# Raiden-Makoto/MLX-VAE

Hardware: AMD Instinct MI355X
Metric: SELFIES sequences/sec (whole node), AR-CVAE training step (higher is better)
Workload: dtype f32

## Files before the change

### include/arcvae_hip.h

```cpp
#ifndef ARCVAE_HIP_H
#define ARCVAE_HIP_H

#include <stdint.h>

#ifdef __cplusplus
extern "C" {
#endif

#define ARCVAE_OK 0
#define ARCVAE_ERR_ARG (-1)
#define ARCVAE_ERR_LAUNCH (-2)
#define ARCVAE_ERR_DEVICE (-3)

#define ARCVAE_GEMM_ACCUMULATE 1
#define ARCVAE_GEMM_TANH 2
#define ARCVAE_GEMM_SPLITK 4
#define ARCVAE_GEMM_NO_SKINNY 8
#define ARCVAE_GEMM_TILE64 16
#define ARCVAE_GEMM_TILE128 32
#define ARCVAE_GEMM_DTANH 64
#define ARCVAE_GEMM_TILE_WIDE 128
#define ARCVAE_GEMM_BF16 256
#define ARCVAE_GEMM_SPLIT3 512
#define ARCVAE_LSTM_RETILE 1
#define ARCVAE_LSTM_BF16 2
#define ARCVAE_LSTM_SPLIT3 4
#define ARCVAE_PERSIST_BF16 2
#define ARCVAE_RS_HALF 16
#define ARCVAE_RS_HALF1 32
#define ARCVAE_DEC_SPLIT3 512
#define ARCVAE_DEC_NO_GPRE 1024
#define ARCVAE_DEC_PART_HEAD 2048
#define ARCVAE_DEC_PART_TAIL 4096
#define ARCVAE_DEC_BF16 256

#ifdef ARCVAE_HIP_BUILD
typedef hipStream_t arcvae_stream_t;
#else
typedef void* arcvae_stream_t;
#endif

int arcvae_abi_version(int* arch_gfx950);

int arcvae_gemm_f32(int transA, int transB, int M, int N, int K, const float* A, int lda,
                    const float* B, int ldb, float* C, int ldc, const float* bias, int flags,
                    arcvae_stream_t stream);

int arcvae_enc_lstm_ws_floats(int B, int T, int H, int L, int flags, long* floats );
int arcvae_transpose_tokens(const int32_t* src_bt, int32_t* dst_tb, int B, int T, arcvae_stream_t stream);
int arcvae_enc_lstm_forward(const int32_t* x_tb, const float* table0, const float* const* Wx,
                            const float* const* Wh, const float* const* bias, float* hseq, float* hseq_t,
                            float* cseq, float* gseq, float* wt, float* wT_bwd , int B, int T, int V,
                            int H, int L, int flags , const long* ws_floats ,
                            void* h_oct ,
                            unsigned long long* trace , arcvae_stream_t stream);
int arcvae_enc_lstm_tiled(int B, int H, int L);
int arcvae_enc_lstm_tiled_for(int B, int H, int L, int flags);
int arcvae_enc_lstm_operand_slots(int B, int T, int H, int L, int flags);
int arcvae_enc_lstm_backward(const float* const* Wx, const float* const* Wh, const float* cseq,
                             const float* gseq, const float* dh_top, int ld_dh_top, float* dG, float* dG_t,
                             float* dcs, float* dxs, float* wT, int B, int T, int H, int L, int s_begin,
// ... 172 lines not shown
```

### mlx-vae_amd/arcvae_hip/_lib.py

```python
from __future__ import annotations

import ctypes as C
import os
from typing import Iterable, Optional, Sequence

import torch

_HERE = os.path.dirname(os.path.abspath(__file__))
LIB_PATH = os.environ.get("ARCVAE_HIP_LIB", os.path.join(_HERE, "libarcvae_hip.so"))

GEMM_ACCUMULATE = 1
GEMM_TANH = 2
GEMM_SPLITK = 4
GEMM_NO_SKINNY = 8
GEMM_BF16 = 256
GEMM_SPLIT3 = 512
LSTM_RETILE = 1
LSTM_BF16 = 2
LSTM_SPLIT3 = 4
RS_HALF, RS_HALF1 = 16, 32
PERSIST_BF16 = 2
DEC_BF16 = 256
DEC_SPLIT3 = 512
DEC_PART_HEAD = 2048
DEC_PART_TAIL = 4096
DEC_NO_GPRE = 1024
WGRAD_BF16 = 128

_vp = C.c_void_p
_i = C.c_int
_f = C.c_float
_d = C.c_double
_l = C.c_long
_pp = C.POINTER(C.c_void_p)
_ip = C.POINTER(C.c_int)
_lp = C.POINTER(C.c_long)

SIGNATURES = {
    "arcvae_abi_version": [_ip],
    "arcvae_gemm_f32": [_i, _i, _i, _i, _i, _vp, _i, _vp, _i, _vp, _i, _vp, _i, _vp],
    "arcvae_transpose_tokens": [_vp, _vp, _i, _i, _vp],
    "arcvae_enc_lstm_ws_floats": [_i, _i, _i, _i, _i, _lp],
    "arcvae_enc_lstm_forward": [_vp, _vp, _pp, _pp, _pp, _vp, _vp, _vp, _vp, _vp, _vp, _i, _i, _i, _i, _i, _i, _lp, _vp, _vp, _vp],
    "arcvae_enc_lstm_tiled": [_i, _i, _i],
    "arcvae_enc_lstm_tiled_for": [_i, _i, _i, _i],
    "arcvae_enc_lstm_operand_slots": [_i, _i, _i, _i, _i],
    "arcvae_dense_stack_ok": [_l, _i, _i],
    "arcvae_dense_stack_ws_floats": [_l, _i, _i, _lp],
    "arcvae_dense_stack_forward": [_pp, _pp, _vp, _vp, _vp, _l, _l, _i, _i, _i, _vp],
    "arcvae_dense_stack_backward": [_vp, _vp, _vp, _vp, _pp, _pp, _vp, _l, _l, _i, _i, _i, _vp],
    "arcvae_enc_lstm_persistent_ok": [_i, _i, _i, _i],
    "arcvae_enc_lstm_forward_persistent": [_vp, _vp, _pp, _pp, _pp, _vp, _vp, _vp, _vp, _l, _vp, _vp, _vp, _i, _i, _i, _i, _i, _i, _vp, _vp],
    "arcvae_enc_prologue": [_vp, _vp, _vp, _l, _vp, _l, _vp, _i, _i, _vp, _vp, _vp, _vp, _vp, _i, _vp, _i, _i, _i, _i, _i, _vp],
    "arcvae_enc_lstm_bwd_persistent_ok": [_i, _i, _i, _i],
    "arcvae_enc_lstm_backward_persistent": [_vp, _vp, _vp, _i, _vp, _vp, _vp, _vp, _vp, _vp, _i, _i, _i, _i, _i, _i, _i, _vp, _vp],
# ... 127 lines not shown
```

### mlx-vae_amd/arcvae_hip/engine.py

```python
from __future__ import annotations

import ctypes as C
import dataclasses
import os
from typing import Dict, Optional, Sequence, Tuple

import numpy as np
import torch

from . import _lib
from ._lib import call, ptr, ptr_array, stream_ptr
from .store import ParamStore

SCALAR_KEYS = ("total_loss", "recon_loss", "kl_loss", "weighted_kl", "collapse_penalty", "prop_loss",
               "weighted_prop_loss", "mutual_info", "mi_penalty")


@dataclasses.dataclass(frozen=True)
class ModelDims:
    V: int
    E: int
    H: int
    Z: int
    C: int
# ... 453 lines not shown
                     ws.B, ws.T, d.H, d.L, s0, s1, chunk_index, (_lib.PERSIST_BF16 if ws.bf16_parts & 1 else 0) | rearmed | hf,
                     ptr(ws.trace_bwd) if not (hf & _lib.RS_HALF1) else C.c_void_p(0), stream_ptr())
            return
        if _lib.load().arcvae_enc_lstm_bwd_persistent_ok(ws.B, ws.T, d.H, d.L) == 1:
            call("arcvae_enc_lstm_backward_persistent", ptr(ws.cseq), ptr(ws.gseq), ptr(ws.dcomb), 2 * d.H, ptr(ws.dG),
                 ptr(ws.dcs), ptr(ws.dxs), ptr(ws.wT), ptr(ws.psync), sig, ws.B, ws.T, d.H, d.L, s0, s1, chunk_index,
                 ptr(ws.trace_bwd), stream_ptr())
            return
        call("arcvae_enc_lstm_backward", self._wx[0], self._wh[0], ptr(ws.cseq), ptr(ws.gseq), ptr(ws.dcomb),
             2 * d.H, ptr(ws.dG), ptr(ws.dG_t), ptr(ws.dcs), ptr(ws.dxs), ptr(ws.wT), ws.B, ws.T, d.H, d.L, s0, s1,
             _lstm_flags(ws),
             _caps(ws), _oct(ws, "dG_oct"), start_signal if start_signal is not None else C.c_void_p(0), ptr(ws.trace_bwd), stream_ptr())

    def wgrad(self, t_lo: int, t_hi: int, first: bool, last: bool, parts: int = 3, table=None) -> None:
        enc, ws, d = self.enc, self.ws, self.d
        if os.environ.get("ARCVAE_DEBUG_SKIP_WGRAD", "0") == "1":
            return
        if self.fused:
            if last and (parts & 2):
                call("arcvae_table_finalize", ptr(ws.dtable0), ptr(enc.p("lstm_layer_0.Wx")), d.E,
                     ptr(enc.p("embedding.weight")), ptr(enc.g("embedding.weight")), ptr(enc.g("lstm_layer_0.Wx")),
                     ptr(enc.g("lstm_layer_0.bias")), d.V, d.E, 4 * d.H, stream_ptr())
            return
        if (ws.bf16_parts & 4) and not self.persistent:
            parts |= _lib.WGRAD_BF16
        elif getattr(ws, "pl_g", None) is not None:
            parts |= 2048 | 4096 | 16
            call("arcvae_enc_lstm_wgrad", ptr(ws.x_tb), ptr(enc.p("embedding.weight")), ptr(enc.p("lstm_layer_0.Wx")),
                 ptr(ws.hseq), ptr(ws.dG), ptr(table if table is not None else ws.dtable0), ptr(ws.onehot),
                 ptr(enc.g("embedding.weight")), self._dwx[0], self._dwh[0], self._dbs[0], ws.B, ws.T, d.V, d.E, d.H, d.L,
                 t_lo, t_hi, int(first), int(last), parts, ptr(ws.pl_h), ptr(ws.pl_g), _caps(ws, ws.pl_h, ws.pl_g), stream_ptr())
# ... 77 lines not shown

def _encoder_backward_gated(plan: EncoderBackwardPlan, ws: Workspace, aux, aux2, run, prologue, after_first,
                            g: Gates, epilogue=None) -> None:
    main = torch.cuda.current_stream()
    nc = len(plan.chunks)
    if nc + 1 > g.STRIDE:
        raise ValueError("too many BPTT chunks for the gate stride")
    if getattr(plan, "fused", False) and nc == 1 and aux2 is not None:
        _encoder_backward_gated_fused(plan, ws, aux, aux2, run, prologue, after_first, g)
        return
    tail_on_side = aux2 is not None and nc >= 2
    table_on_side = tail_on_side and os.environ.get("ARCVAE_TABLE_ON_SIDE", "1") != "0"
    mid_batch = ws is not None and ws.B >= 256 and not (_lib.load().arcvae_enc_lstm_tiled_for(ws.B, plan.d.H, plan.d.L, _lstm_flags(ws)) & 2)
    wx_on_side = table_on_side and os.environ.get("ARCVAE_WX_ON_SIDE", "1" if (plan.persistent or mid_batch) else "0") != "0"
    own_tables = table_on_side and _tables_on_main(plan, ws)

    def pre_zeroed() -> int:
        return 256 if (nc == 2 and ws is not None and getattr(ws, "tables_zeroed", False)) else 0

    def main_seg():
        if prologue:
            prologue()
        plan.heads(1)
        for c, (s0, s1, _t_lo, _t_hi, _first, _last) in enumerate(plan.chunks):
            plan.sweep(s0, s1, g.word(g.P) if c > 0 else g.word(g.H), c)
        g.signal(g.P, g.STRIDE - nc)
        if own_tables:
            _s0, _s1, t_lo_l, t_hi_l, _f, _l = plan.chunks[-1]
            plan.wgrad(t_lo_l, t_hi_l, True, True, 2 | 32 | pre_zeroed(), table=getattr(ws, "dtable1", None))
        if epilogue is not None:
            epilogue()

    if epilogue is not None:
        run("main+finish", main_seg, main, eager_first=False)
    else:
        run("main", main_seg, main)
    if after_first:
        after_first()
    for c, (s0, s1, t_lo, t_hi, first, last) in enumerate(plan.chunks):
        def aux_seg(c=c, t_lo=t_lo, t_hi=t_hi, first=first, last=last):
            heads_early = os.environ.get("ARCVAE_HEADS_EARLY", "0") != "0"
            if c == 0 and heads_early:
                g.wait(g.H, g.NA, 1, 1)
                plan.heads(2)
                g.signal(g.HG, 1)
            g.wait(g.P, g.NA, g.STRIDE, g.STRIDE if last else 2 + c, advance=last)
            if c == 0 and not heads_early:
                plan.heads(2)
                g.signal(g.HG, 1)
            plan.wgrad(t_lo, t_hi, first, last,
                       8 if wx_on_side else (1 if (table_on_side or (last and tail_on_side)) else 3))
            if c == max(nc - 2, 0):
                g.signal(g.Q, 1)
            if last:
                g.signal(g.R, 1 if tail_on_side else 2)

        def side_seg(c=c, t_lo=t_lo, t_hi=t_hi, first=first, last=last):
            if table_on_side:
                g.wait(g.P, g.NS, g.STRIDE, g.STRIDE if last else 2 + c, advance=last)
            else:
                g.wait(g.Q, g.NS, 1, 1)
                g.wait(g.P, g.NS, g.STRIDE, g.STRIDE, advance=True)
            if own_tables:
                plan.wgrad(t_lo, t_hi, True, True, ((4 if wx_on_side else 0) | (0 if last else 2)) | 32 | pre_zeroed())
            else:
                plan.wgrad(t_lo, t_hi, first, last, 6 if wx_on_side else 2)
            if last:
                g.signal(g.R, 1)

        run(f"aux{c}", aux_seg, aux)
        if table_on_side or (last and tail_on_side):
            run(f"aux2_{c}", side_seg, aux2)
    if aux2 is not None and not tail_on_side:
        main.wait_stream(aux2)


NO_GUARDS = (C.c_void_p(0), C.c_void_p(0))

# ... 495 lines not shown
```

### mlx-vae_amd/csrc/gemm.hip

```cpp
#include "ops.h"
#ifdef ARCVAE_PLANE_CLOCK
#include <algorithm>
#include <cstdio>
#include <vector>
#endif
#include "skinny.h"

namespace {

typedef __bf16 bf16x8_t __attribute__((ext_vector_type(8)));
typedef __bf16 bf16x2_t __attribute__((ext_vector_type(2)));
typedef float f32x2_t __attribute__((ext_vector_type(2)));
typedef unsigned u32x4_g __attribute__((ext_vector_type(4)));

__device__ __forceinline__ unsigned split_pk(float a, float b) {
    return __builtin_bit_cast(unsigned, __builtin_convertvector(f32x2_t{a, b}, bf16x2_t));
}

__device__ __forceinline__ void split3(float x0, float x1, unsigned& hi, unsigned& mid, unsigned& lo) {
    hi = split_pk(x0, x1);
    const float r0 = x0 - __uint_as_float(hi << 16), r1 = x1 - __uint_as_float(hi & 0xffff0000u);
    mid = split_pk(r0, r1);
    lo = split_pk(r0 - __uint_as_float(mid << 16), r1 - __uint_as_float(mid & 0xffff0000u));
}
// ... 507 lines not shown
        float* c = p.C + (long)gr * p.ldc + gc;
        if (p.accumulate) v += *c;
        if (p.act == 1) v = tanhf(v);
        if (p.act == 2) { const float t = p.bias[(long)gr * p.ldc + gc]; v *= (1.0f - t * t); }
        *c = v;
    }
}


struct SplitTN {
    const float* A;
    const float* B;
    float* C;
    float* colsum;
    int M, N, K, lda, ldb, ldc, kchunk;
};
#define ARCVAE_SPLIT_GROUP_MAX 8
struct SplitTNGroup {
    SplitTN p[ARCVAE_SPLIT_GROUP_MAX];
    int zoff[ARCVAE_SPLIT_GROUP_MAX + 1];
    int n;
};


template <int MI, int NJ, bool ONE = false>
__device__ __forceinline__ void split_tn_body(const SplitTN& p, const int bx, const int by, const int bz, float* red) {
    constexpr int TT = MI * NJ;
    const int tid = threadIdx.x, lane = tid & 63, wave = tid >> 6, r = lane & 31, h = lane >> 5;
    const int m0 = by * 32 * MI, n0 = bx * 32 * NJ;
    const int kbeg = bz * p.kchunk, kend = min(p.K, kbeg + p.kchunk);
    const int am = m0 + MI * r;
    const bool aok = am < p.M;
    f32x16 acc[MI][NJ];
#pragma unroll
    for (int i = 0; i < MI; ++i)
#pragma unroll
        for (int j = 0; j < NJ; ++j)
#pragma unroll
            for (int q = 0; q < 16; ++q) acc[i][j][q] = 0.f;
    float ra[2][8][MI];
    float rb[2][8][NJ];
    const bool do_cs = p.colsum != nullptr && bx == 0;
    float csum[MI];
#pragma unroll
    for (int i = 0; i < MI; ++i) csum[i] = 0.f;
#define SPLIT_LOAD(BUF, K0)                                                                                       \
    _Pragma("unroll") for (int kk = 0; kk < 8; ++kk) {                                                            \
        const int k = (K0) + 8 * h + kk;                                                                          \
        const bool kok = k < kend;                                                                                \
        if constexpr (MI == 4) {                                                                                  \
            const float4 v = (kok && aok) ? *reinterpret_cast<const float4*>(p.A + (long)k * p.lda + am)          \
                                          : make_float4(0.f, 0.f, 0.f, 0.f);                                      \
            ra[BUF][kk][0] = v.x; ra[BUF][kk][1] = v.y; ra[BUF][kk][MI > 2 ? 2 : 0] = v.z; ra[BUF][kk][MI > 2 ? 3 : 0] = v.w; \
        } else {                                                                                                  \
            const float2 v = (kok && aok) ? *reinterpret_cast<const float2*>(p.A + (long)k * p.lda + am)          \
                                          : make_float2(0.f, 0.f);                                                \
// ... 2 lines not shown
        _Pragma("unroll") for (int j = 0; j < NJ; ++j) {                                                          \
            const int n = n0 + 32 * j + r;                                                                        \
            rb[BUF][kk][j] = (kok && n < p.N) ? p.B[(long)k * p.ldb + n] : 0.f;                                   \
        }                                                                                                         \
    }
#define SPLIT_STEP(BUF, K0)                                                                                       \
    {                                                                                                             \
        if (do_cs) {                                                                                              \
            _Pragma("unroll") for (int kk = 0; kk < 8; ++kk)                                                      \
            _Pragma("unroll") for (int i = 0; i < MI; ++i) csum[i] += ra[BUF][kk][i];                             \
        }                                                                                                         \
        u32x4_g ah[MI], amid[MI], al[MI], bh[NJ], bm[NJ], bl[NJ];                                                 \
        _Pragma("unroll") for (int d = 0; d < 4; ++d) {                                                           \
            unsigned x, y = 0, z = 0;                                                                             \
            _Pragma("unroll") for (int i = 0; i < MI; ++i) {                                                      \
                if constexpr (ONE) x = split_pk(ra[BUF][2 * d][i], ra[BUF][2 * d + 1][i]);                        \
                else split3(ra[BUF][2 * d][i], ra[BUF][2 * d + 1][i], x, y, z);                                   \
                ah[i][d] = x; amid[i][d] = y; al[i][d] = z;                                                       \
            }                                                                                                     \
            _Pragma("unroll") for (int j = 0; j < NJ; ++j) {                                                      \
                if constexpr (ONE) x = split_pk(rb[BUF][2 * d][j], rb[BUF][2 * d + 1][j]);                        \
                else split3(rb[BUF][2 * d][j], rb[BUF][2 * d + 1][j], x, y, z);                                   \
                bh[j][d] = x; bm[j][d] = y; bl[j][d] = z;                                                         \
            }                                                                                                     \
        }                                                                                                         \
        if ((K0) + 128 < kend) { SPLIT_LOAD(BUF, (K0) + 128) }                                                    \
        _Pragma("unroll") for (int i = 0; i < MI; ++i)                                                            \
        _Pragma("unroll") for (int j = 0; j < NJ; ++j) {                                                          \
            const bf16x8_t AH = __builtin_bit_cast(bf16x8_t, ah[i]), AM = __builtin_bit_cast(bf16x8_t, amid[i]),   \
                           AL = __builtin_bit_cast(bf16x8_t, al[i]);                                              \
            const bf16x8_t BH = __builtin_bit_cast(bf16x8_t, bh[j]), BM_ = __builtin_bit_cast(bf16x8_t, bm[j]),    \
                           BL = __builtin_bit_cast(bf16x8_t, bl[j]);                                              \
            f32x16 c = acc[i][j];                                                          \
            if constexpr (!ONE) {                                                                                 \
                c = __builtin_amdgcn_mfma_f32_32x32x16_bf16(AL, BH, c, 0, 0, 0);                                  \
                c = __builtin_amdgcn_mfma_f32_32x32x16_bf16(AH, BL, c, 0, 0, 0);                                  \
                c = __builtin_amdgcn_mfma_f32_32x32x16_bf16(AM, BM_, c, 0, 0, 0);                                 \
                c = __builtin_amdgcn_mfma_f32_32x32x16_bf16(AM, BH, c, 0, 0, 0);                                  \
                c = __builtin_amdgcn_mfma_f32_32x32x16_bf16(AH, BM_, c, 0, 0, 0);                                 \
            }                                                                                                     \
            c = __builtin_amdgcn_mfma_f32_32x32x16_bf16(AH, BH, c, 0, 0, 0);                                      \
            acc[i][j] = c;                                                                                        \
        }                                                                                                         \
    }
    int k0 = kbeg + 16 * wave;
    if (k0 < kend) { SPLIT_LOAD(0, k0) }
    if (k0 + 64 < kend) { SPLIT_LOAD(1, k0 + 64) }
    for (; k0 < kend; k0 += 128) {
        SPLIT_STEP(0, k0)
        if (k0 + 64 < kend) SPLIT_STEP(1, k0 + 64)
    }
#undef SPLIT_STEP
#undef SPLIT_LOAD
    if (do_cs) {
#pragma unroll
        for (int i = 0; i < MI; ++i) {
            const float v = csum[i] + __shfl_xor(csum[i], 32);
            if (h == 0 && aok) atomicAdd(p.colsum + am + i, v);
        }
    }
    const int reg = wave >> 1;
    if (wave & 1) {
#pragma unroll
        for (int i = 0; i < MI; ++i)
#pragma unroll
// ... 30 lines not shown
        for (int q = 0; q < 16; ++q) {
            const int m = m0 + MI * ((q & 3) + 8 * (q >> 2) + 4 * h) + i;
            const float v = red[((0 * TT + t) * 16 + q) * 64 + lane] + red[((1 * TT + t) * 16 + q) * 64 + lane];
            if (m < p.M) atomicAdd(p.C + (long)m * p.ldc + n, v);
        }
    }
}

template <int MI, int NJ, bool ONE = false>
__global__ __launch_bounds__(256) void gemm_split_tn_group_kernel(SplitTNGroup g) {
    extern __shared__ __attribute__((aligned(16))) float split_red[];
    int i = 0;
    while (i + 1 < g.n && (int)blockIdx.z >= g.zoff[i + 1]) ++i;
    const SplitTN& p = g.p[i];
    if ((int)blockIdx.y * 32 * MI >= p.M || (int)blockIdx.x * 32 * NJ >= p.N) return;
    split_tn_body<MI, NJ, ONE>(p, blockIdx.x, blockIdx.y, blockIdx.z - g.zoff[i], split_red);
}

inline bool split_tn_enabled() {
    static const int v = arcvae_env_int("ARCVAE_GEMM_SPLIT", 1);
    return v != 0;
}
inline bool split_tn_ok(int M, int N, const float* A, int lda, const float* B, int ldb) {
    return split_tn_enabled() && (M % 4) == 0 && (lda % 4) == 0 && (reinterpret_cast<uintptr_t>(A) & 15) == 0 && M >= 32 && N >= 16;
}
int launch_split_tn_group(int n, const SplitTN* probs, bool wide, bool one, hipStream_t stream) {
    SplitTNGroup g;
    g.n = n;
    int Mmax = 0, Nmax = 0, ztot = 0;
    static const int target = arcvae_env_int("ARCVAE_SPLIT_BLOCKS", 256);
    for (int i = 0; i < n; ++i) {
// ... 13 lines not shown
        ztot += z;
    }
    g.zoff[n] = ztot;
    for (int i = n; i < ARCVAE_SPLIT_GROUP_MAX; ++i) { g.p[i] = g.p[0]; g.zoff[i + 1] = ztot; }
    dim3 grid(ceil_div(Nmax, 64), ceil_div(Mmax, 32 * mi), ztot);
    const size_t lds = sizeof(float) * 2 * (mi * 2) * 16 * 64;
    if (one) {
        (void)hipFuncSetAttribute((const void*)gemm_split_tn_group_kernel<4, 2, true>, hipFuncAttributeMaxDynamicSharedMemorySize, (int)lds);
        hipLaunchKernelGGL((gemm_split_tn_group_kernel<4, 2, true>), grid, dim3(256), lds, stream, g);
    } else if (mi == 4) {
        (void)hipFuncSetAttribute((const void*)gemm_split_tn_group_kernel<4, 2>, hipFuncAttributeMaxDynamicSharedMemorySize, (int)lds);
        hipLaunchKernelGGL((gemm_split_tn_group_kernel<4, 2>), grid, dim3(256), lds, stream, g);
    } else {
        hipLaunchKernelGGL((gemm_split_tn_group_kernel<2, 2>), grid, dim3(256), lds, stream, g);
    }
    return arcvae_launch_status();
}

struct OctTN {
    const __bf16* A;
    const __bf16* B;
    float* C;
    int K;
    int kchunk;
};
#define ARCVAE_OCT_GROUP_MAX 8
struct OctTNGroup {
    OctTN p[ARCVAE_OCT_GROUP_MAX];
    int zoff[ARCVAE_OCT_GROUP_MAX + 1];
    int n, M, N, ldc;
// ... 128 lines not shown
    GemmP p;
    p.A = A; p.B = B; p.C = C; p.bias = bias;
    p.M = M; p.N = N; p.K = K; p.lda = lda; p.ldb = ldb; p.ldc = ldc;
    p.accumulate = (flags & ARCVAE_GEMM_ACCUMULATE) ? 1 : 0;
    p.act = (flags & ARCVAE_GEMM_TANH) ? 1 : ((flags & ARCVAE_GEMM_DTANH) ? 2 : 0);
    if (p.act == 2 && (!bias || p.accumulate)) return ARCVAE_ERR_ARG;
    p.kchunk = ((K + BK - 1) / BK) * BK;

    const bool ak = !transA, bk = transB != 0;
    const bool bf16_tile_tn = (flags & ARCVAE_GEMM_BF16) && M >= 256 && N >= 256 && K >= 2048;
    if (!bf16_tile_tn)
    if (transA && !transB && (flags & ARCVAE_GEMM_ACCUMULATE) && (flags & ARCVAE_GEMM_SPLITK) && !bias && p.act == 0 &&
        !(flags & (ARCVAE_GEMM_TILE64 | ARCVAE_GEMM_TILE128)) && split_tn_ok(M, N, A, lda, B, ldb)) {
        SplitTN q;
        q.A = A; q.B = B; q.C = C; q.colsum = nullptr; q.M = M; q.N = N; q.K = K; q.lda = lda; q.ldb = ldb; q.ldc = ldc; q.kchunk = 0;
        return launch_split_tn_group(1, &q, (flags & ARCVAE_GEMM_TILE_WIDE) != 0, (flags & ARCVAE_GEMM_BF16) != 0, stream);
    }
    if ((flags & ARCVAE_GEMM_SPLIT3) && !(flags & ARCVAE_GEMM_BF16) && !(transA == 0 && M <= 256)) {
        dim3 grid(ceil_div(N, 64), ceil_div(M, 64), 1);
        if ((flags & ARCVAE_GEMM_SPLITK) && p.act == 0) {
            static const int target3 = arcvae_env_int("ARCVAE_SPLITK_BLOCKS", 512);
            int z = min(ceil_div(target3, (int)(grid.x * grid.y)), max(1, K / 256));
            if (z > 1) {
                p.kchunk = ceil_div(ceil_div(K, z), 64) * 64;
                grid.z = ceil_div(K, p.kchunk);
                if (!p.accumulate && arcvae_zero(C, M, N, ldc, stream) != ARCVAE_OK) return ARCVAE_ERR_LAUNCH;
            }
        }
        if (launch_bf16_tile_t<64, 64, 32, 3>(p, grid, ak, bk, stream)) return arcvae_launch_status();
        p.kchunk = ((K + BK - 1) / BK) * BK;
// ... 64 lines not shown
            return ARCVAE_ERR_ARG;
        p.A = A[i]; p.B = B[i]; p.C = C[i]; p.bias = bias[i];
        p.M = M[i]; p.N = N[i]; p.K = K[i]; p.lda = lda[i]; p.ldb = ldb[i]; p.ldc = ldc[i];
        p.accumulate = (flags[i] & ARCVAE_GEMM_ACCUMULATE) ? 1 : 0;
        p.act = (flags[i] & ARCVAE_GEMM_TANH) ? 1 : ((flags[i] & ARCVAE_GEMM_DTANH) ? 2 : 0);
        if (p.act == 2 && (!bias[i] || p.accumulate)) return ARCVAE_ERR_ARG;
        p.kchunk = 0;
    }
    g.nx0 = ceil_div(N[0], 16);
    dim3 grid(g.nx0 + ceil_div(N[1], 16), ceil_div(max(M[0], M[1]), 16), 1);
    if (transB) hipLaunchKernelGGL(gemm_skinny_pair_kernel<true>, grid, dim3(256), 0, stream, g);
    else hipLaunchKernelGGL(gemm_skinny_pair_kernel<false>, grid, dim3(256), 0, stream, g);
    return arcvae_launch_status();
}

int arcvae_gemm_tn_group_accum(int n, int M, int N, const int* K, const float* const* A, int lda,
                               const float* const* B, int ldb, float* const* C, int ldc, int allow_split,
                               float* const* colsum, hipStream_t stream) {
    if (n <= 0 || n > ARCVAE_GEMM_GROUP_MAX || M <= 0 || N <= 0) return ARCVAE_ERR_ARG;
    auto colsums_by_launch = [&]() -> int {
        for (int i = 0; colsum && i < n; ++i)
            if (colsum[i] && K[i] > 0) {
                const int rc = arcvae_colsum_accum(A[i], K[i], M, lda, colsum[i], 1.0f, stream);
                if (rc) return rc;
            }
        return ARCVAE_OK;
    };
    if ((allow_split & 4) && M >= 256 && N >= 256) {
        for (int i = 0; i < n; ++i) {
            if (K[i] <= 0) continue;
            const int rc = arcvae_gemm_f32(1, 0, M, N, K[i], A[i], lda, B[i], ldb, C[i], ldc, nullptr,
                                           ARCVAE_GEMM_ACCUMULATE | ARCVAE_GEMM_SPLITK | ARCVAE_GEMM_BF16, stream);
            if (rc) return rc;
        }
        return colsums_by_launch();
    }
    if (allow_split & 7) {
        bool ok = true;
        for (int i = 0; i < n; ++i) ok = ok && K[i] > 0 && split_tn_ok(M, N, A[i], lda, B[i], ldb);
        if (ok) {
            const bool ride = arcvae_env_int("ARCVAE_COLSUM_FUSED", 1) != 0;
            SplitTN q[ARCVAE_SPLIT_GROUP_MAX];
            for (int i = 0; i < n; ++i) {
                q[i].A = A[i]; q[i].B = B[i]; q[i].C = C[i]; q[i].colsum = (colsum && ride) ? colsum[i] : nullptr; q[i].M = M; q[i].N = N; q[i].K = K[i];
                q[i].lda = lda; q[i].ldb = ldb; q[i].ldc = ldc; q[i].kchunk = 0;
            }
            const int rc = launch_split_tn_group(n, q, (allow_split & 2) != 0, (allow_split & 4) != 0, stream);
            if (rc || ride) return rc;
            return colsums_by_launch();
        }
    }
    if (allow_split & 8) {
        for (int i = 0; i < n; ++i) {
            if (K[i] <= 0) continue;
            const int rc = arcvae_gemm_f32(1, 0, M, N, K[i], A[i], lda, B[i], ldb, C[i], ldc, nullptr,
                                           ARCVAE_GEMM_ACCUMULATE | ARCVAE_GEMM_SPLITK | ARCVAE_GEMM_SPLIT3 | ARCVAE_GEMM_TILE64, stream);
            if (rc) return rc;
        }
        return colsums_by_launch();
    }
// ... 335 lines not shown
```

### mlx-vae_amd/csrc/lstm.hip

```cpp
#include "ops.h"
#include "skinny.h"
#include "xcd.h"

namespace {

__device__ __forceinline__ int xcd_group_block(int x, int gx, int on) {
    return (on && (gx & 7) == 0) ? (x & 7) * (gx >> 3) + (x >> 3) : x;
}

struct FwdJob {
    const float* xin;
    const float* Wx;
    const float* hprev;
    const float* Wh;
    const float* pre;
    const int32_t* tok;
    const float* cprev;
    float* h;
    float* ht;
    float* c;
    float* gates;
    void* oct;
};
struct FwdArgs {
// ... 3409 lines not shown
                                     hipStream_t stream) {
    if (!x_tb || !emb || !Wx0 || !hseq || !dG || !dtable_ws || !onehot_ws || !dEmb || !dWx || !dWh || !dbias)
        return ARCVAE_ERR_ARG;
    if (t_lo < 0 || t_hi > T || t_lo > t_hi) return ARCVAE_ERR_ARG;
    if ((parts & 2048) && h_oct && dG_oct) {
        if (!ws_floats || ws_floats[0] < (long)L * T * B * H * 3 / 2 || ws_floats[1] < (long)L * T * B * 4 * H * 3 / 2) return ARCVAE_ERR_ARG;
    }
    const int G = 4 * H, TB = T * B;
    const long lH = (long)TB * H, lG = (long)TB * G;
    int rc;
    const bool do_wx = (parts & (1 | 4)) != 0, do_wh = (parts & (1 | 8)) != 0, do_table = (parts & 2) != 0;
    const bool b16 = (parts & 128) != 0;
    const bool exact_f32 = (parts & 16) != 0 && !b16, wide = (parts & 64) != 0;
    const bool do_layers = do_wx || do_wh;
    const int Vp = (V + 3) & ~3;
    if (do_table && first) {
        if (!(parts & 256))
        if (arcvae_zero(dtable_ws, V, G, G, stream) != ARCVAE_OK) return ARCVAE_ERR_LAUNCH;
        const long n = (long)TB * Vp;
        if (!(parts & 32))
        hipLaunchKernelGGL(onehot_kernel, dim3((unsigned)min((long)1024, (n + 255) / 256)), dim3(256), 0, stream, x_tb,
                           TB, V, Vp, onehot_ws);
    }
    if (t_hi > t_lo) {
        const int nt = t_hi - t_lo;
        if (do_layers) {
            const float* Ag[2 * ARCVAE_MAX_LAYERS];
            const float* Bg[2 * ARCVAE_MAX_LAYERS];
            float* Cg[2 * ARCVAE_MAX_LAYERS];
            float* Sg[2 * ARCVAE_MAX_LAYERS];
            int Kg[2 * ARCVAE_MAX_LAYERS];
            int n = 0;
            const int t1 = t_lo > 1 ? t_lo : 1;
            for (int l = 0; l < L; ++l) {
                const float* dGl = dG + l * lG;
                if (do_wh && t_hi > t1) {
                    Ag[n] = dGl + (long)t1 * B * G; Bg[n] = hseq + l * lH + (long)(t1 - 1) * B * H;
                    Cg[n] = dWh[l]; Sg[n] = nullptr; Kg[n] = (t_hi - t1) * B; ++n;
                }
                if (do_wx && l > 0) {
                    Ag[n] = dGl + (long)t_lo * B * G; Bg[n] = hseq + (l - 1) * lH + (long)t_lo * B * H;
                    Cg[n] = dWx[l]; Sg[n] = dbias[l]; Kg[n] = nt * B; ++n;
                }
            }
            if ((parts & 4096) && (parts & 2048) && h_oct && dG_oct) {
                if ((B % 32) != 0 || (H % 64) != 0) return ARCVAE_ERR_ARG;
                __bf16* hp = static_cast<__bf16*>(const_cast<void*>(h_oct));
                __bf16* gp = static_cast<__bf16*>(const_cast<void*>(dG_oct));
                const int h_lo = t_lo > 0 ? t_lo - 1 : 0;
                for (int l = 0; l < L; ++l) {
                    if (do_wh || l > 0)
                        hipLaunchKernelGGL(planes_from_f32_kernel, dim3((unsigned)(((long)B * (G >> 2) + 255) / 256), nt), dim3(256), 0, stream,
                                           dG + l * lG + (long)t_lo * B * G, gp + 3 * (l * lG + (long)t_lo * B * G), (long)B, G);
                    const int a0 = do_wh ? h_lo : t_lo, a1 = (do_wx && l < L - 1) ? t_hi : t_hi - 1;
                    if (a1 > a0 && (do_wh || l < L - 1))
                        hipLaunchKernelGGL(planes_from_f32_kernel, dim3((unsigned)(((long)B * (H >> 2) + 255) / 256), a1 - a0), dim3(256), 0, stream,
                                           hseq + l * lH + (long)a0 * B * H, hp + 3 * (l * lH + (long)a0 * B * H), (long)B, H);
                }
            }
            if ((parts & 2048) && h_oct && dG_oct) {
                if ((B % 32) != 0 || (H % 64) != 0) return ARCVAE_ERR_ARG;
                const void* Ap[2 * ARCVAE_MAX_LAYERS];
                const void* Bp[2 * ARCVAE_MAX_LAYERS];
                int ta[2 * ARCVAE_MAX_LAYERS], tb[2 * ARCVAE_MAX_LAYERS], nts[2 * ARCVAE_MAX_LAYERS];
                for (int i = 0; i < n; ++i) {
                    const long ao = Ag[i] - dG, bo = Bg[i] - hseq;
                    const int la = (int)(ao / lG), lb = (int)(bo / lH);
                    ta[i] = (int)((ao - la * lG) / ((long)B * G)); tb[i] = (int)((bo - lb * lH) / ((long)B * H));
                    nts[i] = Kg[i] / B;
                    Ap[i] = static_cast<const char*>(dG_oct) + 2 * ((long)la * T * 3 * B * G);
                    Bp[i] = static_cast<const char*>(h_oct) + 2 * ((long)lb * T * 3 * B * H);
                }
                for (int i = 0; i < n; i += 8) {
                    rc = arcvae_wgrad_planes_group(n - i < 8 ? n - i : 8, G, H, B, Ap + i, ta + i, Bp + i, tb + i, nts + i, Cg + i, H,
                                                   Sg + i, stream);
// ... 7 lines not shown
                    Bo[i] = static_cast<const char*>(h_oct) + 2 * (Bg[i] - hseq);
                }
                for (int i = 0; i < n; i += 8) {
                    rc = arcvae_wgrad_octet_group(n - i < 8 ? n - i : 8, G, H, Kg + i, Ao + i, Bo + i, Cg + i, H, stream);
                    if (rc) return rc;
                }
                for (int i = 0; i < n; ++i)
                    if (Sg[i]) { rc = arcvae_colsum_accum(Ag[i], Kg[i], G, G, Sg[i], 1.0f, stream); if (rc) return rc; }
            } else
            for (int i = 0; i < n; i += 8) {
                rc = arcvae_gemm_tn_group_accum(n - i < 8 ? n - i : 8, G, H, Kg + i, Ag + i, G, Bg + i, H, Cg + i, H,
                                                (parts & 1024) ? 8 : (exact_f32 ? 0 : (1 | (wide ? 2 : 0) | (b16 ? 4 : 0))), Sg + i, stream);
                if (rc) return rc;
            }
        }
        if (do_table) {
            rc = arcvae_gemm_f32(1, 0, V, G, nt * B, onehot_ws + (long)t_lo * B * Vp, Vp, dG + (long)t_lo * B * G, G,
                                 dtable_ws, G, nullptr,
                                 ARCVAE_GEMM_ACCUMULATE | ARCVAE_GEMM_SPLITK | (exact_f32 ? ARCVAE_GEMM_TILE64 : 0) |
                                     (wide ? ARCVAE_GEMM_TILE_WIDE : 0) | (b16 ? ARCVAE_GEMM_BF16 : 0), stream);
            if (rc) return rc;
        }
    }
    if (last && do_table)
        return arcvae_table_finalize(dtable_ws, Wx0, E, emb, dEmb, dWx[0], dbias[0], V, E, G, stream);
    return arcvae_launch_status();
}
```

Baseline: 69220.

## Fuse last-chunk weight-grad and embedding-table grad into one balanced split-K tail launch

For small batches with two chunks, the final chunk's layer weight-gradient GEMMs and the one-hot table-gradient GEMM now run in a single grouped split-K launch. The split factor per problem is chosen so the total block count fits the compute-unit count, and the kernel uses a 4-deep register buffer plus a two-half accumulation through LDS. Because the one-hot A operand is exactly representable in bf16, the split-bf16 emulation skips the A-low and A-mid MFMA terms, cutting MFMA work per tile. This adds extra LDS traffic and a barrier for the halves path, and changes the scheduling across streams for the last chunk.

```diff
diff --git a/include/arcvae_hip.h b/include/arcvae_hip.h
--- a/include/arcvae_hip.h
+++ b/include/arcvae_hip.h
@@ -22,6 +22,7 @@
 #define ARCVAE_GEMM_TILE_WIDE 128
 #define ARCVAE_GEMM_BF16 256
 #define ARCVAE_GEMM_SPLIT3 512
+#define ARCVAE_GEMM_A_BF16_EXACT 1024
 #define ARCVAE_LSTM_RETILE 1
 #define ARCVAE_LSTM_BF16 2
 #define ARCVAE_LSTM_SPLIT3 4
@@ -45,6 +46,10 @@
 int arcvae_gemm_f32(int transA, int transB, int M, int N, int K, const float* A, int lda,
                     const float* B, int ldb, float* C, int ldc, const float* bias, int flags,
                     arcvae_stream_t stream);
+
+int arcvae_gemm_tn_tail_group(int n, const int* M, const int* N, const int* K, const float* const* A, const int* lda,
+                              const float* const* B, const int* ldb, float* const* C, const int* ldc,
+                              float* const* colsum, const int* a_exact, arcvae_stream_t stream);
 
 int arcvae_enc_lstm_ws_floats(int B, int T, int H, int L, int flags, long* floats );
 int arcvae_transpose_tokens(const int32_t* src_bt, int32_t* dst_tb, int B, int T, arcvae_stream_t stream);
diff --git a/mlx-vae_amd/arcvae_hip/_lib.py b/mlx-vae_amd/arcvae_hip/_lib.py
--- a/mlx-vae_amd/arcvae_hip/_lib.py
+++ b/mlx-vae_amd/arcvae_hip/_lib.py
@@ -26,6 +26,8 @@
 DEC_PART_TAIL = 4096
 DEC_NO_GPRE = 1024
 WGRAD_BF16 = 128
+WGRAD_TAIL = 8192
+GEMM_A_BF16_EXACT = 1024
 
 _vp = C.c_void_p
 _i = C.c_int
@@ -39,6 +41,7 @@
 SIGNATURES = {
     "arcvae_abi_version": [_ip],
     "arcvae_gemm_f32": [_i, _i, _i, _i, _i, _vp, _i, _vp, _i, _vp, _i, _vp, _i, _vp],
+    "arcvae_gemm_tn_tail_group": [_i, _ip, _ip, _ip, _pp, _ip, _pp, _ip, _pp, _ip, _pp, _ip, _vp],
     "arcvae_transpose_tokens": [_vp, _vp, _i, _i, _vp],
     "arcvae_enc_lstm_ws_floats": [_i, _i, _i, _i, _i, _lp],
     "arcvae_enc_lstm_forward": [_vp, _vp, _pp, _pp, _pp, _vp, _vp, _vp, _vp, _vp, _vp, _i, _i, _i, _i, _i, _i, _lp, _vp, _vp, _vp],
diff --git a/mlx-vae_amd/arcvae_hip/engine.py b/mlx-vae_amd/arcvae_hip/engine.py
--- a/mlx-vae_amd/arcvae_hip/engine.py
+++ b/mlx-vae_amd/arcvae_hip/engine.py
@@ -491,7 +491,8 @@
 
     def wgrad(self, t_lo: int, t_hi: int, first: bool, last: bool, parts: int = 3, table=None) -> None:
         enc, ws, d = self.enc, self.ws, self.d
-        if os.environ.get("ARCVAE_DEBUG_SKIP_WGRAD", "0") == "1":
+        skip = os.environ.get("ARCVAE_DEBUG_SKIP_WGRAD", "0")
+        if skip == "1" or (skip == "tail" and t_lo == 0 and t_hi < ws.T):
             return
         if self.fused:
             if last and (parts & 2):
@@ -599,6 +600,10 @@
     mid_batch = ws is not None and ws.B >= 256 and not (_lib.load().arcvae_enc_lstm_tiled_for(ws.B, plan.d.H, plan.d.L, _lstm_flags(ws)) & 2)
     wx_on_side = table_on_side and os.environ.get("ARCVAE_WX_ON_SIDE", "1" if (plan.persistent or mid_batch) else "0") != "0"
     own_tables = table_on_side and _tables_on_main(plan, ws)
+    tail_wgrad = (own_tables and nc == 2 and ws is not None and ws.B <= 64 and not getattr(ws, "bf16_parts", 0) and plan.d.V % 4 == 0
+                  and getattr(ws, "pl_g", None) is None and os.environ.get("ARCVAE_TAIL_WGRAD", "1") != "0")
+    if ws is not None:
+        ws.tail_wgrad = bool(tail_wgrad)
 
     def pre_zeroed() -> int:
         return 256 if (nc == 2 and ws is not None and getattr(ws, "tables_zeroed", False)) else 0
@@ -612,7 +617,8 @@
         g.signal(g.P, g.STRIDE - nc)
         if own_tables:
             _s0, _s1, t_lo_l, t_hi_l, _f, _l = plan.chunks[-1]
-            plan.wgrad(t_lo_l, t_hi_l, True, True, 2 | 32 | pre_zeroed(), table=getattr(ws, "dtable1", None))
+            plan.wgrad(t_lo_l, t_hi_l, True, True, ((1 | _lib.WGRAD_TAIL) if tail_wgrad else 0) | 2 | 32 | pre_zeroed(),
+                       table=getattr(ws, "dtable1", None))
         if epilogue is not None:
             epilogue()
 
@@ -633,8 +639,9 @@
             if c == 0 and not heads_early:
                 plan.heads(2)
                 g.signal(g.HG, 1)
-            plan.wgrad(t_lo, t_hi, first, last,
-                       8 if wx_on_side else (1 if (table_on_side or (last and tail_on_side)) else 3))
+            if not (last and tail_wgrad):
+                plan.wgrad(t_lo, t_hi, first, last,
+                           8 if wx_on_side else (1 if (table_on_side or (last and tail_on_side)) else 3))
             if c == max(nc - 2, 0):
                 g.signal(g.Q, 1)
             if last:
@@ -646,7 +653,9 @@
             else:
                 g.wait(g.Q, g.NS, 1, 1)
                 g.wait(g.P, g.NS, g.STRIDE, g.STRIDE, advance=True)
-            if own_tables:
+            if last and tail_wgrad:
+                pass
+            elif own_tables:
                 plan.wgrad(t_lo, t_hi, True, True, ((4 if wx_on_side else 0) | (0 if last else 2)) | 32 | pre_zeroed())
             else:
                 plan.wgrad(t_lo, t_hi, first, last, 6 if wx_on_side else 2)
diff --git a/mlx-vae_amd/csrc/gemm.hip b/mlx-vae_amd/csrc/gemm.hip
--- a/mlx-vae_amd/csrc/gemm.hip
+++ b/mlx-vae_amd/csrc/gemm.hip
@@ -545,6 +545,7 @@
     float* C;
     float* colsum;
     int M, N, K, lda, ldb, ldc, kchunk;
+    int a_exact;
 };
 #define ARCVAE_SPLIT_GROUP_MAX 8
 struct SplitTNGroup {
@@ -554,7 +555,7 @@
 };
 
 
-template <int MI, int NJ, bool ONE = false>
+template <int MI, int NJ, bool ONE = false, int NB = 2, bool AX = false, bool HALVES = false>
 __device__ __forceinline__ void split_tn_body(const SplitTN& p, const int bx, const int by, const int bz, float* red) {
     constexpr int TT = MI * NJ;
     const int tid = threadIdx.x, lane = tid & 63, wave = tid >> 6, r = lane & 31, h = lane >> 5;
@@ -569,8 +570,8 @@
         for (int j = 0; j < NJ; ++j)
 #pragma unroll
             for (int q = 0; q < 16; ++q) acc[i][j][q] = 0.f;
-    float ra[2][8][MI];
-    float rb[2][8][NJ];
+    float ra[NB][8][MI];
+    float rb[NB][8][NJ];
     const bool do_cs = p.colsum != nullptr && bx == 0;
     float csum[MI];
 #pragma unroll
@@ -603,7 +604,7 @@
         _Pragma("unroll") for (int d = 0; d < 4; ++d) {                                                           \
             unsigned x, y = 0, z = 0;                                                                             \
             _Pragma("unroll") for (int i = 0; i < MI; ++i) {                                                      \
-                if constexpr (ONE) x = split_pk(ra[BUF][2 * d][i], ra[BUF][2 * d + 1][i]);                        \
+                if constexpr (ONE || AX) x = split_pk(ra[BUF][2 * d][i], ra[BUF][2 * d + 1][i]);                  \
                 else split3(ra[BUF][2 * d][i], ra[BUF][2 * d + 1][i], x, y, z);                                   \
                 ah[i][d] = x; amid[i][d] = y; al[i][d] = z;                                                       \
             }                                                                                                     \
@@ -613,7 +614,7 @@
                 bh[j][d] = x; bm[j][d] = y; bl[j][d] = z;                                                         \
             }                                                                                                     \
         }                                                                                                         \
-        if ((K0) + 128 < kend) { SPLIT_LOAD(BUF, (K0) + 128) }                                                    \
+        if ((K0) + 64 * NB < kend) { SPLIT_LOAD(BUF, (K0) + 64 * NB) }                                            \
         _Pragma("unroll") for (int i = 0; i < MI; ++i)                                                            \
         _Pragma("unroll") for (int j = 0; j < NJ; ++j) {                                                          \
             const bf16x8_t AH = __builtin_bit_cast(bf16x8_t, ah[i]), AM = __builtin_bit_cast(bf16x8_t, amid[i]),   \
@@ -622,10 +623,12 @@
                            BL = __builtin_bit_cast(bf16x8_t, bl[j]);                                              \
             f32x16 c = acc[i][j];                                                          \
             if constexpr (!ONE) {                                                                                 \
-                c = __builtin_amdgcn_mfma_f32_32x32x16_bf16(AL, BH, c, 0, 0, 0);                                  \
+                if constexpr (!AX) c = __builtin_amdgcn_mfma_f32_32x32x16_bf16(AL, BH, c, 0, 0, 0);               \
                 c = __builtin_amdgcn_mfma_f32_32x32x16_bf16(AH, BL, c, 0, 0, 0);                                  \
-                c = __builtin_amdgcn_mfma_f32_32x32x16_bf16(AM, BM_, c, 0, 0, 0);                                 \
-                c = __builtin_amdgcn_mfma_f32_32x32x16_bf16(AM, BH, c, 0, 0, 0);                                  \
+                if constexpr (!AX) {                                                                              \
+                    c = __builtin_amdgcn_mfma_f32_32x32x16_bf16(AM, BM_, c, 0, 0, 0);                             \
+                    c = __builtin_amdgcn_mfma_f32_32x32x16_bf16(AM, BH, c, 0, 0, 0);                              \
+                }                                                                                                 \
                 c = __builtin_amdgcn_mfma_f32_32x32x16_bf16(AH, BM_, c, 0, 0, 0);                                 \
             }                                                                                                     \
             c = __builtin_amdgcn_mfma_f32_32x32x16_bf16(AH, BH, c, 0, 0, 0);                                      \
@@ -633,11 +636,41 @@
         }                                                                                                         \
     }
     int k0 = kbeg + 16 * wave;
-    if (k0 < kend) { SPLIT_LOAD(0, k0) }
-    if (k0 + 64 < kend) { SPLIT_LOAD(1, k0 + 64) }
-    for (; k0 < kend; k0 += 128) {
-        SPLIT_STEP(0, k0)
-        if (k0 + 64 < kend) SPLIT_STEP(1, k0 + 64)
+#pragma unroll
+    for (int s = 0; s < NB; ++s)
+        if (k0 + 64 * s < kend) { SPLIT_LOAD(s, k0 + 64 * s) }
+    float* const half = red + wave * (TT * 16 * 64);
+    const int kmid = HALVES ? kbeg + (kend - kbeg) / 2 : kend;
+    bool halved = false;
+#pragma unroll 1
+    for (int part = 0; part < (HALVES ? 2 : 1); ++part) {
+        const int kstop = part == 0 ? kmid : kend;
+        const bool any = k0 < kstop;
+        for (; k0 < kstop; k0 += 64 * NB) {
+#pragma unroll
+            for (int s = 0; s < NB; ++s)
+                if (k0 + 64 * s < kend) SPLIT_STEP(s, k0 + 64 * s)
+        }
+        if (HALVES && part == 0 && any && k0 < kend) {
+            halved = true;
+#pragma unroll
+            for (int i = 0; i < MI; ++i)
+#pragma unroll
+                for (int j = 0; j < NJ; ++j)
+#pragma unroll
+                    for (int q = 0; q < 16; ++q) { half[((i * NJ + j) * 16 + q) * 64 + lane] = acc[i][j][q]; acc[i][j][q] = 0.f; }
+        }
+    }
+    if constexpr (HALVES) {
+        if (halved) {
+#pragma unroll
+            for (int i = 0; i < MI; ++i)
+#pragma unroll
+                for (int j = 0; j < NJ; ++j)
+#pragma unroll
+                    for (int q = 0; q < 16; ++q) acc[i][j][q] += half[((i * NJ + j) * 16 + q) * 64 + lane];
+        }
+        __syncthreads();
     }
 #undef SPLIT_STEP
 #undef SPLIT_LOAD
@@ -698,7 +731,25 @@
     while (i + 1 < g.n && (int)blockIdx.z >= g.zoff[i + 1]) ++i;
     const SplitTN& p = g.p[i];
     if ((int)blockIdx.y * 32 * MI >= p.M || (int)blockIdx.x * 32 * NJ >= p.N) return;
-    split_tn_body<MI, NJ, ONE>(p, blockIdx.x, blockIdx.y, blockIdx.z - g.zoff[i], split_red);
+    if (!ONE && p.a_exact) split_tn_body<MI, NJ, ONE, 2, true>(p, blockIdx.x, blockIdx.y, blockIdx.z - g.zoff[i], split_red);
+    else split_tn_body<MI, NJ, ONE>(p, blockIdx.x, blockIdx.y, blockIdx.z - g.zoff[i], split_red);
+}
+
+struct SplitTNTail {
+    SplitTN p[ARCVAE_SPLIT_GROUP_MAX];
+    int boff[ARCVAE_SPLIT_GROUP_MAX + 1];
+    int nx[ARCVAE_SPLIT_GROUP_MAX], nz[ARCVAE_SPLIT_GROUP_MAX];
+    int n;
+};
+__global__ __launch_bounds__(256) void gemm_split_tn_tail_kernel(SplitTNTail g) {
+    extern __shared__ __attribute__((aligned(16))) float split_red[];
+    int i = 0;
+    while (i + 1 < g.n && (int)blockIdx.x >= g.boff[i + 1]) ++i;
+    const SplitTN& p = g.p[i];
+    const int local = blockIdx.x - g.boff[i], tile = local / g.nz[i], bz = local - tile * g.nz[i];
+    const int by = tile / g.nx[i], bx = tile - by * g.nx[i];
+    if (p.a_exact) split_tn_body<4, 2, false, 4, true, true>(p, bx, by, bz, split_red);
+    else split_tn_body<4, 2, false, 4, false, true>(p, bx, by, bz, split_red);
 }
 
 inline bool split_tn_enabled() {
@@ -742,6 +793,56 @@
     } else {
         hipLaunchKernelGGL((gemm_split_tn_group_kernel<2, 2>), grid, dim3(256), lds, stream, g);
     }
+    return arcvae_launch_status();
+}
+
+int launch_split_tn_tail(int n, const SplitTN* probs, hipStream_t stream) {
+    static const int ncu = [] {
+        int dev = 0, v = 0;
+        if (hipGetDevice(&dev) != hipSuccess || hipDeviceGetAttribute(&v, hipDeviceAttributeMultiprocessorCount, dev) != hipSuccess) v = 0;
+        return v > 0 ? v : 256;
+    }();
+    SplitTNTail g;
+    g.n = n;
+    int tiles[ARCVAE_SPLIT_GROUP_MAX], zmax[ARCVAE_SPLIT_GROUP_MAX], z[ARCVAE_SPLIT_GROUP_MAX];
+    long cost[ARCVAE_SPLIT_GROUP_MAX];
+    for (int i = 0; i < n; ++i) {
+        g.p[i] = probs[i];
+        g.nx[i] = ceil_div(probs[i].N, 64);
+        tiles[i] = g.nx[i] * ceil_div(probs[i].M, 128);
+        cost[i] = (long)probs[i].K * (probs[i].a_exact ? 3 : 6);
+        zmax[i] = max(1, probs[i].K / 256);
+        z[i] = 1;
+    }
+    auto blocks_at = [&](long cap, int* zz) {
+        int total = 0;
+        for (int j = 0; j < n; ++j) {
+            zz[j] = (int)min((long)zmax[j], (cost[j] + cap - 1) / cap);
+            total += tiles[j] * zz[j];
+        }
+        return total;
+    };
+    long best = 0;
+    for (int i = 0; i < n; ++i)
+        for (int zi = 1; zi <= zmax[i]; ++zi) {
+            const long cap = (cost[i] + zi - 1) / zi;
+            int zz[ARCVAE_SPLIT_GROUP_MAX];
+            if (blocks_at(cap, zz) > ncu) break;
+            if (best == 0 || cap < best) { best = cap; for (int j = 0; j < n; ++j) z[j] = zz[j]; }
+        }
+    int btot = 0;
+    for (int i = 0; i < n; ++i) {
+        SplitTN& p = g.p[i];
+        p.kchunk = ceil_div(ceil_div(p.K, z[i]), 64) * 64;
+        g.nz[i] = ceil_div(p.K, p.kchunk);
+        g.boff[i] = btot;
+        btot += tiles[i] * g.nz[i];
+    }
+    g.boff[n] = btot;
+    for (int i = n; i < ARCVAE_SPLIT_GROUP_MAX; ++i) { g.p[i] = g.p[0]; g.nx[i] = g.nx[0]; g.nz[i] = g.nz[0]; g.boff[i + 1] = btot; }
+    const size_t lds = sizeof(float) * 4 * 8 * 16 * 64;
+    (void)hipFuncSetAttribute((const void*)gemm_split_tn_tail_kernel, hipFuncAttributeMaxDynamicSharedMemorySize, (int)lds);
+    hipLaunchKernelGGL(gemm_split_tn_tail_kernel, dim3(btot), dim3(256), lds, stream, g);
     return arcvae_launch_status();
 }
 
@@ -900,6 +1001,7 @@
         !(flags & (ARCVAE_GEMM_TILE64 | ARCVAE_GEMM_TILE128)) && split_tn_ok(M, N, A, lda, B, ldb)) {
         SplitTN q;
         q.A = A; q.B = B; q.C = C; q.colsum = nullptr; q.M = M; q.N = N; q.K = K; q.lda = lda; q.ldb = ldb; q.ldc = ldc; q.kchunk = 0;
+        q.a_exact = (flags & ARCVAE_GEMM_A_BF16_EXACT) ? 1 : 0;
         return launch_split_tn_group(1, &q, (flags & ARCVAE_GEMM_TILE_WIDE) != 0, (flags & ARCVAE_GEMM_BF16) != 0, stream);
     }
     if ((flags & ARCVAE_GEMM_SPLIT3) && !(flags & ARCVAE_GEMM_BF16) && !(transA == 0 && M <= 256)) {
@@ -994,6 +1096,22 @@
     return arcvae_launch_status();
 }
 
+extern "C" int arcvae_gemm_tn_tail_group(int n, const int* M, const int* N, const int* K, const float* const* A, const int* lda,
+                                         const float* const* B, const int* ldb, float* const* C, const int* ldc,
+                                         float* const* colsum, const int* a_exact, hipStream_t stream) {
+    if (n <= 0 || n > ARCVAE_SPLIT_GROUP_MAX || !M || !N || !K || !A || !lda || !B || !ldb || !C || !ldc) return ARCVAE_ERR_ARG;
+    SplitTN q[ARCVAE_SPLIT_GROUP_MAX];
+    for (int i = 0; i < n; ++i) {
+        if (M[i] <= 0 || N[i] <= 0 || K[i] <= 0 || !A[i] || !B[i] || !C[i] || lda[i] < M[i] || ldb[i] < N[i] || ldc[i] < N[i] ||
+            (M[i] % 4) != 0 || (lda[i] % 4) != 0 || !aligned16(A[i]) || M[i] < 32 || N[i] < 16)
+            return ARCVAE_ERR_ARG;
+        q[i].A = A[i]; q[i].B = B[i]; q[i].C = C[i]; q[i].colsum = colsum ? colsum[i] : nullptr;
+        q[i].M = M[i]; q[i].N = N[i]; q[i].K = K[i]; q[i].lda = lda[i]; q[i].ldb = ldb[i]; q[i].ldc = ldc[i]; q[i].kchunk = 0;
+        q[i].a_exact = (a_exact && a_exact[i]) ? 1 : 0;
+    }
+    return launch_split_tn_tail(n, q, stream);
+}
+
 int arcvae_gemm_tn_group_accum(int n, int M, int N, const int* K, const float* const* A, int lda,
                                const float* const* B, int ldb, float* const* C, int ldc, int allow_split,
                                float* const* colsum, hipStream_t stream) {
@@ -1023,7 +1141,7 @@
             SplitTN q[ARCVAE_SPLIT_GROUP_MAX];
             for (int i = 0; i < n; ++i) {
                 q[i].A = A[i]; q[i].B = B[i]; q[i].C = C[i]; q[i].colsum = (colsum && ride) ? colsum[i] : nullptr; q[i].M = M; q[i].N = N; q[i].K = K[i];
-                q[i].lda = lda; q[i].ldb = ldb; q[i].ldc = ldc; q[i].kchunk = 0;
+                q[i].lda = lda; q[i].ldb = ldb; q[i].ldc = ldc; q[i].kchunk = 0; q[i].a_exact = 0;
             }
             const int rc = launch_split_tn_group(n, q, (allow_split & 2) != 0, (allow_split & 4) != 0, stream);
             if (rc || ride) return rc;
diff --git a/mlx-vae_amd/csrc/lstm.hip b/mlx-vae_amd/csrc/lstm.hip
--- a/mlx-vae_amd/csrc/lstm.hip
+++ b/mlx-vae_amd/csrc/lstm.hip
@@ -3447,6 +3447,8 @@
     const bool exact_f32 = (parts & 16) != 0 && !b16, wide = (parts & 64) != 0;
     const bool do_layers = do_wx || do_wh;
     const int Vp = (V + 3) & ~3;
+    const bool tail = (parts & 8192) != 0;
+    if (tail && ((parts & (16 | 128 | 1024 | 2048)) || (V % 4) != 0)) return ARCVAE_ERR_ARG;
     if (do_table && first) {
         if (!(parts & 256))
         if (arcvae_zero(dtable_ws, V, G, G, stream) != ARCVAE_OK) return ARCVAE_ERR_LAUNCH;
@@ -3476,6 +3478,17 @@
                     Cg[n] = dWx[l]; Sg[n] = dbias[l]; Kg[n] = nt * B; ++n;
                 }
             }
+            if (tail) {
+                if (n + 1 > 8) return ARCVAE_ERR_ARG;
+                int Mg[8], Ng[8], lda[8], ldb[8], ldc[8], ax[8];
+                for (int i = 0; i < n; ++i) { Mg[i] = G; Ng[i] = H; lda[i] = G; ldb[i] = H; ldc[i] = H; ax[i] = 0; }
+                if (do_table) {
+                    Ag[n] = onehot_ws + (long)t_lo * B * Vp; Bg[n] = dG + (long)t_lo * B * G; Cg[n] = dtable_ws; Sg[n] = nullptr;
+                    Kg[n] = nt * B; Mg[n] = V; Ng[n] = G; lda[n] = Vp; ldb[n] = G; ldc[n] = G; ax[n] = 1; ++n;
+                }
+                rc = n > 0 ? arcvae_gemm_tn_tail_group(n, Mg, Ng, Kg, Ag, lda, Bg, ldb, Cg, ldc, Sg, ax, stream) : ARCVAE_OK;
+                if (rc) return rc;
+            }
             if ((parts & 4096) && (parts & 2048) && h_oct && dG_oct) {
                 if ((B % 32) != 0 || (H % 64) != 0) return ARCVAE_ERR_ARG;
                 __bf16* hp = static_cast<__bf16*>(const_cast<void*>(h_oct));
@@ -3491,7 +3504,8 @@
                                            hseq + l * lH + (long)a0 * B * H, hp + 3 * (l * lH + (long)a0 * B * H), (long)B, H);
                 }
             }
-            if ((parts & 2048) && h_oct && dG_oct) {
+            if (tail) {
+            } else if ((parts & 2048) && h_oct && dG_oct) {
                 if ((B % 32) != 0 || (H % 64) != 0) return ARCVAE_ERR_ARG;
                 const void* Ap[2 * ARCVAE_MAX_LAYERS];
                 const void* Bp[2 * ARCVAE_MAX_LAYERS];
@@ -3529,10 +3543,10 @@
                 if (rc) return rc;
             }
         }
-        if (do_table) {
+        if (do_table && !(tail && do_layers)) {
             rc = arcvae_gemm_f32(1, 0, V, G, nt * B, onehot_ws + (long)t_lo * B * Vp, Vp, dG + (long)t_lo * B * G, G,
                                  dtable_ws, G, nullptr,
-                                 ARCVAE_GEMM_ACCUMULATE | ARCVAE_GEMM_SPLITK | (exact_f32 ? ARCVAE_GEMM_TILE64 : 0) |
+                                 ARCVAE_GEMM_ACCUMULATE | ARCVAE_GEMM_SPLITK | ARCVAE_GEMM_A_BF16_EXACT | (exact_f32 ? ARCVAE_GEMM_TILE64 : 0) |
                                      (wide ? ARCVAE_GEMM_TILE_WIDE : 0) | (b16 ? ARCVAE_GEMM_BF16 : 0), stream);
             if (rc) return rc;
         }
```

New measurement: 67830. -2.0%, worse.
